# wulibingbinglin/COMET-Pose-Estimation

Hardware: AMD Instinct MI355X
Metric: sequences/sec (BxT frames) COMET fwd+bwd, T=16 512^2 (higher is better)
Workload: dtype bf16; 1 GPU; train_e2epose2.py fwd+bwd (COMET tracker+DINOv2+head, loss, backward, grad all-reduce, clip 1.0, AdamW) -- BASELINE configs[2]; global_batch=8, seq_len=16, image=512, tracks=512, parallelism=dp1

## Files before the change

### comet-pose-estimation_amd/csrc/gemm.hip

```cpp
#include <cstdio>
#include <cstdlib>
#include <type_traits>

#include "common.hpp"

namespace comet {


namespace {

constexpr int BM = 128, BN = 128, NT = 256;

struct Epi {
  const float* bias; int bias_mode; int64_t sb0, sb1;
  const void* resid; int64_t ldr, sr0, sr1; float beta;
  void* aux; int64_t ldaux, sx0, sx1;
  float alpha; int act;
  int vec;
  int wide = 0;
  int prio = 0;
  int bpark = 0;
  int raster = 0;
  const __bf16* gpre = nullptr; int64_t ldg = 0; float* dcol = nullptr;
};
// ... 527 lines not shown
    for (int e = 0; e < 4; ++e)
      if (col0 + e < N) epi_store<TC>(epi, Cb, ldc, R, X, bias, row, col0 + e, s[e]);
  }
}

template <typename TC, int NT16, int KC>
__global__ void __launch_bounds__(256)
gemm_skinny_kernel(const __bf16* __restrict__ A, int64_t lda, const __bf16* __restrict__ B, int64_t ldb,
                   TC* __restrict__ C, int64_t ldc, int64_t M, int N, int K, Epi epi) {
  const int lane = threadIdx.x & 63, li = lane & 15, g = lane >> 4;
  bf16x8 bf[NT16][KC];
#pragma unroll
  for (int nt = 0; nt < NT16; ++nt)
#pragma unroll
    for (int c = 0; c < KC; ++c) {
      const int n = nt * 16 + li, k0 = 32 * c + 8 * g;
      bf[nt][c] = (n < N && k0 < K) ? *reinterpret_cast<const bf16x8*>(B + (int64_t)n * ldb + k0) : bf16x8{};
    }
  float bias4[NT16][4];
#pragma unroll
  for (int nt = 0; nt < NT16; ++nt)
#pragma unroll
    for (int r = 0; r < 4; ++r) {
      const int n = nt * 16 + 4 * g + r;
      bias4[nt][r] = (epi.bias && n < N) ? epi.bias[n] : 0.f;
    }
  const TC* R = reinterpret_cast<const TC*>(epi.resid);
  const int64_t wave = ((int64_t)blockIdx.x * 256 + threadIdx.x) >> 6;
  const int64_t nwaves = ((int64_t)gridDim.x * 256) >> 6;
  for (int64_t m0 = wave * 16; m0 < M; m0 += nwaves * 16) {
    const int64_t m = m0 + li;
    const bool mok = m < M;
    f32x4 acc[NT16];
#pragma unroll
    for (int nt = 0; nt < NT16; ++nt) acc[nt] = f32x4{0.f, 0.f, 0.f, 0.f};
#pragma unroll
    for (int c = 0; c < KC; ++c) {
      const int k0 = 32 * c + 8 * g;
      const bf16x8 a = (mok && k0 < K) ? *reinterpret_cast<const bf16x8*>(A + m * lda + k0) : bf16x8{};
#pragma unroll
      for (int nt = 0; nt < NT16; ++nt) acc[nt] = __builtin_amdgcn_mfma_f32_16x16x32_bf16(bf[nt][c], a, acc[nt], 0, 0, 0);
    }
    if (!mok) continue;
#pragma unroll
    for (int nt = 0; nt < NT16; ++nt) {
      const int n0 = nt * 16 + 4 * g;
      if (n0 >= N) continue;
      float v[4];
#pragma unroll
      for (int r = 0; r < 4; ++r) v[r] = epi.alpha * acc[nt][r] + bias4[nt][r];
      apply_act_n<4>(epi.act, v);
      if (R) {
        float rr[4];
        load4(R + m * epi.ldr + n0, rr);
#pragma unroll
        for (int r = 0; r < 4; ++r) v[r] += epi.beta * rr[r];
      }
      store4(C + m * ldc + n0, v);
    }
  }
}

bool skinny_ok(const comet_gemm_args& a) {
  if (a.dtype_ab != COMET_BF16 || a.layout_a != 0 || a.layout_b != 0 || a.convert_a || a.convert_b) return false;
  if (a.batch[0] * a.batch[1] != 1 || a.aux != nullptr || (a.bias && a.bias_mode != 1)) return false;
  if (a.n % 16 != 0 || a.n > 64 || a.k % 8 != 0 || a.k > 256 || a.m < 16384) return false;
  const int es = a.dtype_c == COMET_F32 ? 4 : 2;
  auto al = [](const void* p, int bytes) { return p == nullptr || (uintptr_t)p % bytes == 0; };
  if (!al(a.a, 16) || a.lda % 8 != 0 || !al(a.b, 16) || a.ldb % 8 != 0) return false;
  if ((uintptr_t)a.c % (4 * es) != 0 || a.ldc % 4 != 0) return false;
  if (a.resid && ((uintptr_t)a.resid % (4 * es) != 0 || a.ldr % 4 != 0)) return false;
  return true;
}

template <typename TC>
int launch_skinny(const comet_gemm_args& a, hipStream_t s) {
  Epi e{a.bias, a.bias_mode, 0, 0, a.resid, a.ldr, 0, 0, a.beta, nullptr, 0, 0, 0, a.alpha, a.act, 0};
  const int64_t tiles = cdiv(a.m, 16);
  int64_t blocks = cdiv(tiles, 4 * 8);
  if (blocks > 4096) blocks = 4096;
  const int nt = (int)(a.n / 16), kc = (int)cdiv(a.k, 32);
#define SK(NT, KC)                                                                                          \
  hipLaunchKernelGGL((gemm_skinny_kernel<TC, NT, KC>), dim3((unsigned)blocks), dim3(256), 0, s,            \
                     (const __bf16*)a.a, a.lda, (const __bf16*)a.b, a.ldb, (TC*)a.c, a.ldc, a.m, (int)a.n, (int)a.k, e)
#define SK_K(NT) do { if (kc == 1) SK(NT, 1); else if (kc == 2) SK(NT, 2); else if (kc <= 4) SK(NT, 4); else SK(NT, 8); } while (0)
  if (nt == 1) SK_K(1); else if (nt == 2) SK_K(2); else if (nt == 3) SK_K(3); else SK_K(4);
#undef SK_K
#undef SK
  COMET_CHECK_LAUNCH("comet_gemm (skinny)");
  return COMET_OK;
}

namespace big {
constexpr int BM = 256, BK = 64, NT = 512;
constexpr int ASTAGE = BM * BK;
constexpr int CPW = 64;

typedef __attribute__((address_space(3))) void lds_void;

template <int ROWS>
__device__ __forceinline__ void glds_tile(const __bf16* __restrict__ src, int64_t ld, int64_t r0, int64_t rmax,
                                          int64_t k0, __bf16* __restrict__ img, int wid, int lane) {
  constexpr int PER_WAVE = ROWS / 8 / 8;
#pragma unroll
  for (int i = 0; i < PER_WAVE; ++i) {
    const int c = wid * PER_WAVE + i;
    const int row = c * 8 + (lane >> 3), pch = lane & 7;
    const int lch = pch ^ ((row >> 1) & 7);
    int64_t gr = r0 + row;
    gr = gr < rmax ? gr : rmax - 1;
    const __bf16* gp = src + gr * ld + k0 + lch * 8;
    __builtin_amdgcn_global_load_lds((const void*)gp, (lds_void*)(img + c * 512), 16, 0, 0);
  }
}

__device__ __forceinline__ bf16x8 frag(const __bf16* __restrict__ img, int row, int lchunk) {
  return *reinterpret_cast<const bf16x8*>(img + row * 64 + ((lchunk ^ ((row >> 1) & 7)) << 3));
}

__device__ __forceinline__ int tswz(int k) { return (k & 3) | (((k >> 3) & 1) << 2); }

template <int ROWS>
__device__ __forceinline__ void glds_tile_t(const __bf16* __restrict__ src, int64_t ld, int64_t r0, int64_t rmax,
                                            int64_t k0, __bf16* __restrict__ img, int wid, int lane) {
  constexpr int CPR = ROWS / 8;
  constexpr int KPC = 64 / CPR;
  constexpr int PER_WAVE = ROWS / 8 / 8;
#pragma unroll
  for (int i = 0; i < PER_WAVE; ++i) {
    const int c = wid * PER_WAVE + i;
    const int krow = c * KPC + lane / CPR, pch = lane % CPR;
    const int lch = pch ^ (tswz(krow) << 1);
    int64_t gr = r0 + lch * 8;
    gr = gr < rmax ? gr : rmax - 8;
    const __bf16* gp = src + (k0 + krow) * ld + gr;
    __builtin_amdgcn_global_load_lds((const void*)gp, (lds_void*)(img + c * 512), 16, 0, 0);
  }
}

typedef __attribute__((address_space(3))) s16x4 lds_s16x4g;

template <int ROWS>
__device__ __forceinline__ bf16x8 frag_t(const __bf16* __restrict__ img, int rbase, int s, int lane) {
  const int g = lane >> 4, q = (lane >> 2) & 3, p = lane & 3;
  const int u = rbase >> 4;
  const int k0 = s * 32 + 8 * g + q, k1 = k0 + 4;
  const __bf16* a0 = img + k0 * ROWS + ((u ^ tswz(k0)) << 4) + 4 * p;
  const __bf16* a1 = img + k1 * ROWS + ((u ^ tswz(k1)) << 4) + 4 * p;
  const s16x4 v0 = __builtin_amdgcn_ds_read_tr16_b64_v4i16((lds_s16x4g*)(a0));
  const s16x4 v1 = __builtin_amdgcn_ds_read_tr16_b64_v4i16((lds_s16x4g*)(a1));
  return __builtin_bit_cast(bf16x8, __builtin_shufflevector(v0, v1, 0, 1, 2, 3, 4, 5, 6, 7));
}

template <typename TC, int BN, int LA, int LB, bool SPLIT, int VAR = 0, bool DACT = false>
__global__ void __launch_bounds__(NT, 1)
gemm_big_kernel(const __bf16* __restrict__ A, int64_t lda, const __bf16* __restrict__ B, int64_t ldb,
                TC* __restrict__ C, int64_t ldc, int64_t M, int64_t N, int64_t K, int tiles_n, Epi epi,
                Split sp) {
  constexpr int WN = BN / 64, WM = 8 / WN;
  constexpr int MI = BM / WM / 16;
  constexpr int BSTAGE = BN * BK;
  constexpr int STAGING = 2 * ASTAGE + 2 * BSTAGE, PARKING = 8 * 64 * CPW * 2;
  __shared__ __attribute__((aligned(1024))) __bf16 smem[STAGING > PARKING ? STAGING : PARKING];
  const int tile = xcd_remap(blockIdx.x, gridDim.x);
  const int tm = tile / tiles_n, tn = tile % tiles_n;
  const int64_t m0 = (int64_t)tm * BM, n0 = (int64_t)tn * BN;
  const int lane = threadIdx.x & 63, wid = threadIdx.x >> 6;
  const int wr = wid / WN, wc = wid % WN;
  const int li = lane & 15, g = lane >> 4;
  __bf16* const Asm = smem;
  __bf16* const Bsm = smem + 2 * ASTAGE;

  f32x4 acc[MI][4];
#pragma unroll
  for (int i = 0; i < MI; ++i)
#pragma unroll
    for (int j = 0; j < 4; ++j) acc[i][j] = f32x4{0.f, 0.f, 0.f, 0.f};

  int64_t kbeg = 0, kend = K;
  if (SPLIT) {
    kbeg = (int64_t)blockIdx.y * sp.kchunk;
    kend = kbeg + sp.kchunk < K ? kbeg + sp.kchunk : K;
  }
  const int nk = (int)((kend - kbeg) / BK);
  auto load_tiles = [&](int64_t k0, int stage) {
    if constexpr (LA == 0) glds_tile<BM>(A, lda, m0, M, k0, Asm + stage * ASTAGE, wid, lane);
    else glds_tile_t<BM>(A, lda, m0, M, k0, Asm + stage * ASTAGE, wid, lane);
    if constexpr (LB == 0) glds_tile<BN>(B, ldb, n0, N, k0, Bsm + stage * BSTAGE, wid, lane);
    else glds_tile_t<BN>(B, ldb, n0, N, k0, Bsm + stage * BSTAGE, wid, lane);
  };
  auto afrag = [&](const __bf16* img, int rbase, int s) {
    if constexpr (LA == 0) return frag(img, rbase + li, 4 * s + g);
    else return frag_t<BM>(img, rbase, s, lane);
  };
  auto bfrag = [&](const __bf16* img, int rbase, int s) {
    if constexpr (LB == 0) return frag(img, rbase + li, 4 * s + g);
    else return frag_t<BN>(img, rbase, s, lane);
  };
  if (nk > 0) load_tiles(kbeg, 0);

  auto body = [&](int kt, auto load_next) {
    constexpr bool LOAD = decltype(load_next)::value;
    const int cur = kt & 1;
    asm volatile("s_waitcnt vmcnt(0)" ::: "memory");
    asm volatile("s_barrier" ::: "memory");
    const __bf16* a_img = Asm + cur * ASTAGE;
    const __bf16* b_img = Bsm + cur * BSTAGE;
    bf16x8 a0[MI], b0[4], a1[MI], b1[4];
    if constexpr (LOAD && VAR != 3) load_tiles(kbeg + (int64_t)(kt + 1) * BK, cur ^ 1);
#pragma unroll
    for (int j = 0; j < 4; ++j) b0[j] = bfrag(b_img, wc * 64 + j * 16, 0);
#pragma unroll
    for (int i = 0; i < MI; ++i) a0[i] = afrag(a_img, wr * (MI * 16) + i * 16, 0);
    if constexpr (LOAD && VAR == 3) load_tiles(kbeg + (int64_t)(kt + 1) * BK, cur ^ 1);
#pragma unroll
    for (int j = 0; j < 4; ++j) b1[j] = bfrag(b_img, wc * 64 + j * 16, 1);
#pragma unroll
    for (int i = 0; i < MI; ++i) a1[i] = afrag(a_img, wr * (MI * 16) + i * 16, 1);
    if constexpr (VAR == 1) __builtin_amdgcn_s_setprio(1);
#pragma unroll
    for (int i = 0; i < MI; ++i)
#pragma unroll
      for (int j = 0; j < 4; ++j)
        acc[i][j] = __builtin_amdgcn_mfma_f32_16x16x32_bf16(a0[i], b0[j], acc[i][j], 0, 0, 0);
#pragma unroll
    for (int i = 0; i < MI; ++i)
#pragma unroll
      for (int j = 0; j < 4; ++j)
        acc[i][j] = __builtin_amdgcn_mfma_f32_16x16x32_bf16(a1[i], b1[j], acc[i][j], 0, 0, 0);
    if constexpr (VAR == 1) __builtin_amdgcn_s_setprio(0);
    constexpr int RD = MI * (LA ? 2 : 1) + 4 * (LB ? 2 : 1);
    if constexpr (VAR == 3) {
      constexpr int NG = LOAD ? BM / 64 + BN / 64 : 0;
      __builtin_amdgcn_sched_group_barrier(0x100, RD, 0);
#pragma unroll
      for (int q = 0; q < NG; ++q) {
        __builtin_amdgcn_sched_group_barrier(0x020, 1, 0);
        __builtin_amdgcn_sched_group_barrier(0x008, 2, 0);
      }
#pragma unroll
      for (int q = 0; q < RD; ++q) {
        __builtin_amdgcn_sched_group_barrier(0x100, 1, 0);
        __builtin_amdgcn_sched_group_barrier(0x008, 1, 0);
      }
      __builtin_amdgcn_sched_group_barrier(0x008, 8 * MI - 2 * NG - RD, 0);
    } else if constexpr (VAR != 2) {
      constexpr int PAIRS = RD < 4 * MI ? RD : 4 * MI;
      __builtin_amdgcn_sched_group_barrier(0x100, RD, 0);
#pragma unroll
      for (int q = 0; q < PAIRS; ++q) {
        __builtin_amdgcn_sched_group_barrier(0x100, 1, 0);
        __builtin_amdgcn_sched_group_barrier(0x008, 2, 0);
      }
      __builtin_amdgcn_sched_group_barrier(0x100, RD - PAIRS, 0);
      __builtin_amdgcn_sched_group_barrier(0x008, 8 * MI - 2 * PAIRS, 0);
    }
  };
  for (int kt = 0; kt + 1 < nk; ++kt) body(kt, std::true_type{});
  if (nk > 0) body(nk - 1, std::false_type{});
  asm volatile("s_waitcnt lgkmcnt(0)" ::: "memory");
  asm volatile("s_barrier" ::: "memory");

  float* park = reinterpret_cast<float*>(smem) + wid * 64 * CPW;
  const TC* R = reinterpret_cast<const TC*>(epi.resid);
  TC* X = reinterpret_cast<TC*>(epi.aux);
  const int rq = g * 4;
  const int cg = lane & 7, rb = lane >> 3;
  const int64_t col0 = n0 + wc * 64 + cg * 8;
  float bc[8], cs[8];
#pragma unroll
  for (int e = 0; e < 8; ++e) {
    bc[e] = (epi.bias && epi.bias_mode == 1 && col0 + e < N) ? epi.bias[col0 + e] : 0.f;
    cs[e] = 0.f;
  }
#pragma unroll
  for (int h = 0; h < MI / 4; ++h) {
    if (h) asm volatile("s_waitcnt lgkmcnt(0)" ::: "memory");
#pragma unroll
    for (int i = 0; i < 4; ++i)
#pragma unroll
      for (int j = 0; j < 4; ++j)
#pragma unroll
        for (int r = 0; r < 4; ++r) {
          const int row = i * 16 + rq + r, col = j * 16 + li;
          park[row * CPW + (col ^ ((row & 3) << 4))] = acc[h * 4 + i][j][r];
        }
#pragma unroll 2
    for (int q = 0; q < 8; ++q) {
      const int rl = rb + 8 * q;
      const int64_t row = m0 + wr * (MI * 16) + h * 64 + rl;
      float v[8];
      load8(park + rl * CPW + ((cg * 8) ^ ((rl & 3) << 4)), v);
      if (row >= M || col0 >= N) continue;
      if constexpr (SPLIT) {
        float* W = sp.ws + (int64_t)blockIdx.y * M * N + row * N + col0;
        if (N % 8 == 0) {
          store8(W, v);
        } else {
#pragma unroll
          for (int e = 0; e < 8; ++e)
            if (col0 + e < N) W[e] = v[e];
        }
        continue;
      }
      if constexpr (DACT) {
        float pr[8];
        load8(epi.gpre + row * epi.ldg + col0, pr);
#pragma unroll
        for (int e = 0; e < 8; ++e) {
          const float gq = to_f32(from_f32<TC>(epi.alpha * v[e] * gelu_grad_fast(pr[e])));
          v[e] = gq;
          cs[e] += gq;
        }
        store8(C + row * ldc + col0, v);
        continue;
      }
      const float br = (epi.bias && epi.bias_mode == 2) ? epi.bias[row] : 0.f;
#pragma unroll
      for (int e = 0; e < 8; ++e) v[e] = epi.alpha * v[e] + bc[e] + br;
      if (epi.vec && col0 + 8 <= N) {
        if (X) store8(X + row * epi.ldaux + col0, v);
        apply_act_n<8>(epi.act, v);
        if (R) {
          float rr[8];
          load8(R + row * epi.ldr + col0, rr);
#pragma unroll
          for (int e = 0; e < 8; ++e) v[e] += epi.beta * rr[e];
        }
        store8(C + row * ldc + col0, v);
      } else {
#pragma unroll
        for (int e = 0; e < 8; ++e) {
          const int64_t col = col0 + e;
          if (col >= N) break;
          float o = v[e];
          if (X) X[row * epi.ldaux + col] = from_f32<TC>(o);
          o = apply_act(epi.act, o);
          if (R) o += epi.beta * to_f32(R[row * epi.ldr + col]);
          C[row * ldc + col] = from_f32<TC>(o);
        }
      }
    }
  }
  if constexpr (DACT) {
    if (epi.dcol != nullptr) {
#pragma unroll
      for (int e = 0; e < 8; ++e) {
        float x = cs[e];
        x += __shfl_xor(x, 8, 64);
        x += __shfl_xor(x, 16, 64);
        x += __shfl_xor(x, 32, 64);
        cs[e] = x;
      }
      if (rb == 0 && col0 < N) {
#pragma unroll
        for (int e = 0; e < 8; ++e) atomicAdd(epi.dcol + col0 + e, cs[e]);
      }
    }
  }
}
}

namespace w4 {
constexpr int BK = 64;
constexpr int WGM = 8;

__device__ __forceinline__ void tile_rc(int L, int tiles_m, int tiles_n, int& tm, int& tn) {
  const int gsz = WGM * tiles_n, grp = L / gsz, rem = L - grp * gsz;
  const int rows = min(WGM, tiles_m - grp * WGM);
  tm = grp * WGM + rem % rows;
  tn = rem / rows;
}

typedef __attribute__((address_space(3))) void lds_void;

constexpr int SG_MFMA = 0x008, SG_DSR = 0x100, SG_VMR = 0x020;

#ifdef COMET_GEMM_STAMPS
constexpr int ST_WG = 256, ST_TILES = 64;
__device__ unsigned long long g_stamps[ST_WG * ST_TILES * 8];
__device__ __forceinline__ void stamp(int bid, int wid, int tile, int ph) {
  const unsigned long long t = __builtin_amdgcn_s_memtime();
  if (wid == 0 && bid < ST_WG && tile < ST_TILES && (threadIdx.x & 63) == 0)
    g_stamps[((bid * ST_TILES + tile) << 3) + ph + (threadIdx.x & 63)] = t;
}
__device__ __forceinline__ void kstamp(int bid, int wid, int tile, int ph) {
  __builtin_amdgcn_sched_barrier(0);
  const unsigned long long t = __builtin_amdgcn_s_memtime();
  if ((wid == 0 || wid == 4) && bid < ST_WG && tile < 32 && (threadIdx.x & 63) == 0)
    g_stamps[((bid * ST_TILES + tile + (wid == 4 ? 32 : 0)) << 3) + ph] = t;
  __builtin_amdgcn_sched_barrier(0);
}
#define COMET_STAMP(tile, ph) stamp(bid, wid, (tile), (ph))
#define COMET_KSTAMP(tile, ph) kstamp(bid, wid, (tile), (ph))
#else
#define COMET_STAMP(tile, ph) ((void)0)
#define COMET_KSTAMP(tile, ph) ((void)0)
#endif

struct RowLN {
  __bf16* y16; int64_t ldy; float eps_y;
  __bf16* z16; int64_t ldz; const float* zw; const float* zb; float eps_z;
  int raw_c;
};

template <typename TC, int ACT, bool HASR, int NW, int TBM, int TBN, bool LN = false, bool PING = false>
__global__ void __launch_bounds__(NW * 64, 1)
gemm_w4_kernel(const __bf16* __restrict__ A, int64_t lda, const __bf16* __restrict__ B, int64_t ldb,
               TC* __restrict__ C, int64_t ldc, int64_t M, int64_t N, int64_t K, int tiles_n, int ntiles,
               Epi epi, RowLN ln) {
  constexpr int WN = NW / 2;
  constexpr int WROWS = TBM / 2;
  constexpr int WCOLS = TBN / WN;
  constexpr int MI = WROWS / 16;
  constexpr int NI = WCOLS / 16;
  constexpr int ASTAGE = TBM * BK;
  constexpr int BUF = (TBM + TBN) * BK;
  constexpr int APC = TBM / 8;
  constexpr int PA = APC >= NW ? APC / NW : 1, PB = TBN / 8 / NW;
  constexpr int NMF = MI * NI;
  constexpr int NRD = MI + NI;
  constexpr bool BPARK = std::is_same<TC, __bf16>::value && !HASR && !LN && WCOLS == 64 && ACT == COMET_ACT_NONE;
  constexpr bool PARK = std::is_same<TC, float>::value || (WCOLS % 64 == 0 && ACT == COMET_ACT_NONE && !BPARK);
  constexpr bool WIDE = !PARK && !BPARK && !HASR && std::is_same<TC, __bf16>::value && (NI % 2 == 0);
  constexpr int BSLAB = 16 * WCOLS;
  constexpr int BPARK_B = BPARK ? NW * 2 * BSLAB : 0;
  constexpr bool PSWZ = (WCOLS & (WCOLS - 1)) == 0;
  constexpr int PPITCH = PSWZ ? WCOLS : WCOLS + 4;
  constexpr int PARK_F = PARK ? NW * 8 * PPITCH : 0;
  auto pswz = [](int r) { return PSWZ ? ((r & 7) | ((r & 2) << 2)) : 0; };
  static_assert(!LN || (PARK && std::is_same<TC, float>::value), "row LN epilogue: parked f32 outputs only");
  static_assert(!LN || !BPARK, "row LN epilogue: no bf16 park");
  constexpr int STATS_F = LN ? 2 * TBM * WN : 0;
  constexpr int PARK_ELEMS = 2 * PARK_F > BPARK_B ? 2 * PARK_F : BPARK_B;
#ifdef COMET_GEMM_NO_AR
  constexpr bool AR = false;
#else
  constexpr bool AR = 2 * (3 * ASTAGE + 2 * TBN * BK + PARK_ELEMS + 2 * STATS_F) <= 160 * 1024 && TBM <= 128;
#endif
  constexpr int NA = AR ? 3 : 2;
  constexpr int BSTAGE = TBN * BK;
  constexpr int BRING = NA * ASTAGE;
  constexpr int RING = NA * ASTAGE + 2 * BSTAGE;
  constexpr int XA = AR ? PA : 0;
  static_assert(AR || RING == 2 * BUF, "ring layout");
  __shared__ __attribute__((aligned(1024))) __bf16 smem[RING + PARK_ELEMS + 2 * STATS_F];
  const int lane = threadIdx.x & 63;
  const int wid = __builtin_amdgcn_readfirstlane(threadIdx.x >> 6);
  const int wr = wid / WN, wc = wid % WN;
  const int li = lane & 15, g = lane >> 4;
  const int nk = (int)(K / BK);
  const int G = gridDim.x, bid = blockIdx.x;
  const int tiles_m = ntiles / tiles_n;
  const bool single = ntiles <= G;
  int off = single ? xcd_remap(bid, G) : (bid & 7) * (G >> 3) + (bid >> 3), strd = G, lim = ntiles;
  if (!single && epi.raster && (G & 7) == 0) {
    const int x = bid & 7, per = ntiles >> 3, rem = ntiles & 7, base = x * per + min(x, rem);
    lim = base + per + (x < rem ? 1 : 0);
    off = base + (bid >> 3);
    strd = G >> 3;
  }
  const int my_tiles = single ? 1 : (off < lim ? (lim - off + strd - 1) / strd : 0);
  const int T = my_tiles * nk;
  if (T == 0) return;

#ifdef COMET_APIECE_WRAP_ALL
  const int pieca = (wid * PA) % APC;
#else
  const int pieca = APC < NW ? (wid * PA) % APC : wid * PA;
#endif
  const int prowa = pieca * 8 + (lane >> 3), prowb = wid * PB * 8 + (lane >> 3);
  int la_it = 0, la_kt = 0, lb_it = 0, lb_kt = 0;
  const __bf16* ldA = A;
  const __bf16* ldB = B;
  int offA[PA], offB[PB];
  auto lch = [&](int r) { return ((lane & 7) ^ ((r >> 1) & 7)) * 8; };
  auto set_tile_a = [&](int it) {
    int tm, tn;
    tile_rc(off + it * strd, tiles_m, tiles_n, tm, tn);
    const int m0 = tm * TBM;
    ldA = A + (int64_t)m0 * lda;
#pragma unroll
    for (int p = 0; p < PA; ++p)
      offA[p] = (min(m0 + prowa + p * 8, (int)M - 1) - m0) * (int)lda + lch(prowa + p * 8);
  };
  auto set_tile_b = [&](int it) {
    int tm, tn;
    tile_rc(off + it * strd, tiles_m, tiles_n, tm, tn);
    const int n0 = tn * TBN;
    ldB = B + (int64_t)n0 * ldb;
#pragma unroll
    for (int p = 0; p < PB; ++p)
      offB[p] = (min(n0 + prowb + p * 8, (int)N - 1) - n0) * (int)ldb + lch(prowb + p * 8);
  };
  auto issue_a = [&](int slot) {
    const __bf16* pa = ldA + la_kt * BK;
#pragma unroll
    for (int p = 0; p < PA; ++p)
      __builtin_amdgcn_global_load_lds((const void*)(pa + offA[p]), (lds_void*)(smem + slot * ASTAGE + (pieca + p) * 512), 16, 0, 0);
  };
  auto issue_b = [&](int slot) {
    const __bf16* pb = ldB + lb_kt * BK;
#pragma unroll
    for (int p = 0; p < PB; ++p)
      __builtin_amdgcn_global_load_lds((const void*)(pb + offB[p]),
                                       (lds_void*)(smem + BRING + slot * BSTAGE + (wid * PB + p) * 512), 16, 0, 0);
  };
  auto issue_cur = [&](int aslot, int bslot) {
    if constexpr (AR) {
      issue_b(bslot);
      issue_a(aslot);
    } else {
// ... 1335 lines not shown
constexpr int PXP = CI + 8;
constexpr int MAXW = 128;
constexpr int RP = (MAXW + 2) * PXP;
typedef __attribute__((ext_vector_type(16))) float f32x16;

template <typename TC>
__global__ void __launch_bounds__(512, 1)
conv3_rows_kernel(const __bf16* __restrict__ x, int h, int w, const __bf16* __restrict__ wt, int64_t ldw,
                  TC* __restrict__ y, int64_t ldy, int64_t rows_total, int rows_per, Epi epi) {
  extern __shared__ __attribute__((aligned(16))) __bf16 lds[];
  __bf16* Ws = lds;
  __bf16* Xr = lds + CO * WP;
  constexpr int NT = 512;
  const int tid = threadIdx.x, lane = tid & 63, wid = tid >> 6;
  const int r = lane & 31, hh = lane >> 5;
  const int pb = wid & 3, cb = wid >> 2;
  const int64_t R0 = (int64_t)blockIdx.x * rows_per;
  const int64_t R1 = R0 + rows_per < rows_total ? R0 + rows_per : rows_total;
  if (R0 >= R1) return;

  for (int i = tid; i < CO * (KK / 8); i += NT) {
    const int co = i / (KK / 8), c = i % (KK / 8);
    *reinterpret_cast<uint4*>(Ws + co * WP + 8 * c) = *reinterpret_cast<const uint4*>(wt + (int64_t)co * ldw + 8 * c);
  }
  for (int i = tid; i < 4 * 2 * (CI / 8); i += NT) {
    const int slot = i / (2 * (CI / 8)), rem = i % (2 * (CI / 8));
    const int px = (rem / (CI / 8)) ? w + 1 : 0;
    *reinterpret_cast<uint4*>(Xr + slot * RP + px * PXP + 8 * (rem % (CI / 8))) = uint4{0, 0, 0, 0};
  }
  const int nch = w * (CI / 8);
  constexpr int MAXCH = MAXW * (CI / 8) / NT;
  uint4 st[MAXCH];
  auto rload = [&](int64_t ni, int row) {
    const bool in = row >= 0 && row < h;
    const __bf16* src = x + ((ni * h + (in ? row : 0)) * (int64_t)w) * CI;
#pragma unroll
    for (int i = 0; i < MAXCH; ++i) {
      const int idx = tid + i * NT;
      st[i] = (in && idx < nch) ? *reinterpret_cast<const uint4*>(src + (int64_t)idx * 8) : uint4{0, 0, 0, 0};
    }
  };
  auto rstore = [&](int row) {
    COMET_DASSERT(row >= -1 && row <= h);
    __bf16* dst = Xr + ((row + 1) & 3) * RP;
#pragma unroll
    for (int i = 0; i < MAXCH; ++i) {
      const int idx = tid + i * NT;
      if (idx < nch) *reinterpret_cast<uint4*>(dst + ((idx >> 3) + 1) * PXP + 8 * (idx & 7)) = st[i];
    }
  };
  const int px = pb * 32 + r;
  const bool pxok = px < w;
  const __bf16* wbase = Ws + (cb * 32 + r) * WP + 8 * hh;

  int64_t ni = R0 / h;
  int oy = (int)(R0 % h);
  for (int dr = -1; dr <= 1; ++dr) {
    rload(ni, oy + dr);
    rstore(oy + dr);
  }
  __syncthreads();
  for (int64_t R = R0; R < R1; ++R) {
    const bool next_same = R + 1 < R1 && oy + 1 < h;
    if (next_same) rload(ni, oy + 2);
    f32x16 acc = f32x16{};
#pragma unroll
    for (int ky = 0; ky < 3; ++ky) {
      const __bf16* xb = Xr + ((oy + ky) & 3) * RP + px * PXP + 8 * hh;
#pragma unroll
      for (int kx = 0; kx < 3; ++kx)
#pragma unroll
        for (int c = 0; c < CI; c += 16) {
          const bf16x8 bx = *reinterpret_cast<const bf16x8*>(xb + kx * PXP + c);
          const bf16x8 aw = *reinterpret_cast<const bf16x8*>(wbase + (ky * 3 + kx) * CI + c);
          acc = __builtin_amdgcn_mfma_f32_32x32x16_bf16(aw, bx, acc, 0, 0, 0);
        }
    }
    TC* yrow = y + (R * w + px) * ldy;
    const TC* rrow = reinterpret_cast<const TC*>(epi.resid) + (R * w + px) * epi.ldr;
#pragma unroll
    for (int u = 0; u < 4; u += 2) {
      float v[2][4];
#pragma unroll
      for (int e = 0; e < 2; ++e)
#pragma unroll
        for (int q = 0; q < 4; ++q) {
          const int co = 32 * cb + 8 * (u + e) + 4 * hh + q;
          v[e][q] = apply_act(epi.act, acc[4 * (u + e) + q] + (epi.bias ? epi.bias[co] : 0.f));
        }
      float o[8];
#pragma unroll
      for (int q = 0; q < 4; ++q) {
        const auto sw = __builtin_amdgcn_permlane32_swap(__float_as_uint(v[0][q]), __float_as_uint(v[1][q]), false, false);
        o[q] = __uint_as_float(sw[0]);
        o[4 + q] = __uint_as_float(sw[1]);
      }
      const int co0 = 32 * cb + 8 * u + 8 * hh;
      if (pxok) {
        if (epi.resid) {
          float rv[8];
          load8(rrow + co0, rv);
#pragma unroll
          for (int q = 0; q < 8; ++q) o[q] += epi.beta * rv[q];
        }
        store8(yrow + co0, o);
      }
    }
    if (next_same) rstore(oy + 2);
    __syncthreads();
    ++oy;
    if (oy == h && R + 1 < R1) {
      ++ni;
      oy = 0;
      for (int dr = -1; dr <= 1; ++dr) {
        rload(ni, dr);
        rstore(dr);
      }
      __syncthreads();
    }
  }
}
}

template <typename TC>
bool conv_rows_ok(const comet_conv_args& a) {
  if (getenv("COMET_CONV_NO_ROWS") != nullptr) return false;
  if (a.kh != 3 || a.kw != 3 || a.stride != 1 || a.pad != 1 || a.c != cr::CI || a.cout != cr::CO) return false;
  if (a.w > cr::MAXW || a.w < 96 || a.w % 32 != 0 || a.ldw < cr::KK || a.ldw % 8 != 0 || a.n * a.h < 256) return false;
  const uintptr_t al = 8 * sizeof(TC) >= 16 ? 16 : 8 * sizeof(TC);
  if ((uintptr_t)a.y % al != 0 || a.ldy % 8 != 0) return false;
  if (a.resid && ((uintptr_t)a.resid % al != 0 || a.ldr % 8 != 0)) return false;
  return true;
}

template <typename TC>
int launch_conv_rows(const comet_conv_args& a, hipStream_t s) {
  Epi e{a.bias, a.bias ? 1 : 0, 0, 0, a.resid, a.ldr, 0, 0, a.beta, nullptr, 0, 0, 0, 1.f, a.act, 1};
  const int64_t rows = a.n * a.h;
  int grid = num_cus();
  const int rows_per = (int)cdiv(rows, grid);
  grid = (int)cdiv(rows, rows_per);
  const size_t lds = (size_t)(cr::CO * cr::WP + 4 * cr::RP) * sizeof(__bf16);
  static bool attr = false;
  if (!attr) {
    (void)hipFuncSetAttribute((const void*)cr::conv3_rows_kernel<TC>, hipFuncAttributeMaxDynamicSharedMemorySize, (int)lds);
    attr = true;
  }
  hipLaunchKernelGGL((cr::conv3_rows_kernel<TC>), dim3((unsigned)grid), dim3(512), lds, s, (const __bf16*)a.x,
                     (int)a.h, (int)a.w, (const __bf16*)a.weight, a.ldw, (TC*)a.y, a.ldy, rows, rows_per, e);
  COMET_CHECK_LAUNCH("comet_conv2d_nhwc (3x3 rows in LDS)");
  return COMET_OK;
}

template <typename TC>
int launch_conv(const comet_conv_args& a, hipStream_t s) {
  const int64_t oh = (a.h + 2 * a.pad - a.kh) / a.stride + 1, ow = (a.w + 2 * a.pad - a.kw) / a.stride + 1;
  const int64_t M = a.n * oh * ow, N = a.cout, K = (int64_t)a.kh * a.kw * a.c;
  const int64_t tiles_m = cdiv(M, BM), tiles_n = cdiv(N, BN);
  COMET_CHECK_ARG(tiles_m * tiles_n < (1ll << 31), "comet_conv2d_nhwc: too many tiles");
  const int vec = a.cout % 8 == 0 && (uintptr_t)a.y % 32 == 0 && a.ldy % 8 == 0 &&
                  (a.resid == nullptr || ((uintptr_t)a.resid % 32 == 0 && a.ldr % 8 == 0));
  Epi e{a.bias, a.bias ? 1 : 0, 0, 0, a.resid, a.ldr, 0, 0, a.beta, nullptr, 0, 0, 0, 1.f, a.act, vec};
  bf::ConvGeo g{reinterpret_cast<const __bf16*>(a.x), (int)a.h, (int)a.w, (int)a.c, a.kw, a.stride, a.pad,
                (int)oh, (int)ow};
  if (conv_rows_ok<TC>(a)) return launch_conv_rows<TC>(a, s);
  const int64_t kcs = cdiv(K, 32);
  const bool stem = a.cout == 64 && kcs > 8 && kcs <= 13 && getenv("COMET_CONV_NO_STEM") == nullptr;
  if (a.cout % 16 == 0 && a.cout <= 64 && ((a.cout / 16) * kcs <= 32 || stem) && kcs <= 16 && M >= 16384 &&
      (uintptr_t)a.y % (4 * sizeof(TC)) == 0 && a.ldy % 4 == 0 && getenv("COMET_CONV_NO_SKINNY") == nullptr &&
      (a.resid == nullptr || ((uintptr_t)a.resid % (4 * sizeof(TC)) == 0 && a.ldr % 4 == 0)))
    return launch_conv_skinny<TC>(a, M, (int)oh, (int)ow, (int)K, s);
  Split sp{nullptr, K};
  if (N <= 64 && getenv("COMET_CONV_NO_N64") == nullptr)
    hipLaunchKernelGGL((bf::gemm_bf16_kernel<TC, 0, 0, bf::K_BF16_VEC, bf::K_BF16_VEC, false, true, true>),
                       dim3((unsigned)(tiles_m * tiles_n), 1, 1), dim3(NT), 0, s,
                       nullptr, 0, 0, 0, reinterpret_cast<const __bf16*>(a.weight), a.ldw, 0, 0,
                       reinterpret_cast<TC*>(a.y), a.ldy, 0, 0, M, N, K, 1, (int)tiles_n, e, sp, g);
  else
    hipLaunchKernelGGL((bf::gemm_bf16_kernel<TC, 0, 0, bf::K_BF16_VEC, bf::K_BF16_VEC, false, true>),
                       dim3((unsigned)(tiles_m * tiles_n), 1, 1), dim3(NT), 0, s,
                       nullptr, 0, 0, 0, reinterpret_cast<const __bf16*>(a.weight), a.ldw, 0, 0,
                       reinterpret_cast<TC*>(a.y), a.ldy, 0, 0, M, N, K, 1, (int)tiles_n, e, sp, g);
  COMET_CHECK_LAUNCH("comet_conv2d_nhwc");
  return COMET_OK;
}

}

}

extern "C" int comet_conv2d_nhwc(const comet_conv_args* args, void* stream) {
  using namespace comet;
  COMET_CHECK_ARG(args != nullptr, "comet_conv2d_nhwc: null args");
  const comet_conv_args& a = *args;
  COMET_CHECK_ARG(a.dtype == COMET_BF16, "comet_conv2d_nhwc: x/weight must be bf16 (use im2col + comet_gemm for f32)");
  COMET_CHECK_ARG(a.c > 0 && a.c % 8 == 0, "comet_conv2d_nhwc: channels must be a positive multiple of 8");
  COMET_CHECK_ARG(a.n > 0 && a.h > 0 && a.w > 0 && a.cout > 0 && a.kh > 0 && a.kw > 0 && a.stride > 0 && a.pad >= 0,
                  "comet_conv2d_nhwc: bad geometry");
  COMET_CHECK_ARG(a.h + 2 * a.pad >= a.kh && a.w + 2 * a.pad >= a.kw, "comet_conv2d_nhwc: kernel larger than padded input");
  COMET_CHECK_ARG(a.ldw >= (int64_t)a.kh * a.kw * a.c && a.ldw % 8 == 0, "comet_conv2d_nhwc: ldw < kh*kw*c or not a multiple of 8");
  COMET_CHECK_ARG(a.x && a.weight && a.y, "comet_conv2d_nhwc: null pointer");
  COMET_CHECK_ARG((uintptr_t)a.x % 16 == 0 && (uintptr_t)a.weight % 16 == 0, "comet_conv2d_nhwc: x/weight must be 16-byte aligned");
  COMET_CHECK_ARG(a.n * a.h * a.w * a.c < (1ll << 40), "comet_conv2d_nhwc: input too large");
  hipStream_t s = as_stream(stream);
  if (a.dtype_y == COMET_BF16) return launch_conv<__bf16>(a, s);
  if (a.dtype_y == COMET_F32) return launch_conv<float>(a, s);
  set_error("comet_conv2d_nhwc: bad dtype_y");
  return COMET_EINVAL;
}

extern "C" int comet_gemm_workspace(const comet_gemm_args* args, int64_t* bytes) {
  using namespace comet;
  const int rc = validate(args);
  if (rc != COMET_OK) return rc;
  COMET_CHECK_ARG(bytes != nullptr, "comet_gemm_workspace: null bytes");
  *bytes = plan_workspace(*args, make_plan(*args));
  return COMET_OK;
}

extern "C" int comet_gemm_plan(const comet_gemm_args* args, int64_t* bytes, int32_t* plan) {
  using namespace comet;
  const int rc = validate(args);
  if (rc != COMET_OK) return rc;
  COMET_CHECK_ARG(bytes != nullptr && plan != nullptr, "comet_gemm_plan: null output");
  const Plan p = make_plan(*args);
  *bytes = plan_workspace(*args, p);
  plan[0] = p.kind;
  plan[1] = p.bn;
  plan[2] = (p.kind == 3 || p.kind == 4) ? p.bm : p.splits;
  return COMET_OK;
}

static bool rowln_ok(const comet_gemm_args& a, const comet_rowln_args* ln) {
  using namespace comet;
  if (!pp_ok(a) || a.dtype_c != COMET_F32 || a.resid == nullptr || a.aux != nullptr || a.act != COMET_ACT_NONE) return false;
  if (a.n != 384 && a.n != 256) return false;
  int tbm, tbn;
  pp_tile_base(a, tbm, tbn);
  if (tbn != a.n) return false;
  auto a16 = [](const void* p) { return p == nullptr || (uintptr_t)p % 16 == 0; };
  if (!a16(a.bias)) return false;
  if (ln == nullptr) return true;
  auto b4 = [](const void* p, int64_t ld) { return p == nullptr || ((uintptr_t)p % 8 == 0 && ld % 4 == 0); };
  if (!b4(ln->y16, ln->ldy) || !b4(ln->z16, ln->ldz)) return false;
  if (ln->z16 != nullptr && (ln->zw == nullptr || ln->zb == nullptr)) return false;
  if (!a16(ln->zw) || !a16(ln->zb)) return false;
  return true;
}

extern "C" int comet_gemm_rowln_workspace(const comet_gemm_args* args, int64_t* bytes) {
  using namespace comet;
  COMET_CHECK_ARG(bytes != nullptr, "comet_gemm_rowln_workspace: null bytes");
  *bytes = 0;
  const int rc = validate(args);
  if (rc != COMET_OK) return rc;
  if (rowln_ok(*args, nullptr)) {
    if (const int sp = rowln_splits(*args)) *bytes = rowln_ws_bytes(*args, sp);
  }
  return COMET_OK;
}

extern "C" int comet_gemm_rowln_ok(const comet_gemm_args* args) {
  using namespace comet;
  if (args == nullptr || validate(args) != COMET_OK) return 0;
  return rowln_ok(*args, nullptr) ? 1 : 0;
}

extern "C" int comet_gemm_rowln(const comet_gemm_args* args, const comet_rowln_args* ln, void* stream) {
  using namespace comet;
  const int rc = validate(args);
  if (rc != COMET_OK) return rc;
  COMET_CHECK_ARG(ln != nullptr && args->a && args->b && args->c, "comet_gemm_rowln: null operand");
  COMET_CHECK_ARG(rowln_ok(*args, ln), "comet_gemm_rowln: not eligible (bf16 k-contiguous operands, K % 64 == 0, "
                                       "M >= 4096, N in {256, 384}, f32 output with a residual, no activation / aux)");
  if (args->m == 0) return COMET_OK;
  w4::RowLN r{reinterpret_cast<__bf16*>(ln->y16), ln->ldy, ln->eps_y, reinterpret_cast<__bf16*>(ln->z16), ln->ldz,
              ln->zw, ln->zb, ln->eps_z, ln->raw_c};
  return launch_pp_rowln(*args, r, as_stream(stream));
}

namespace comet {
namespace {
bool dact_ok(const comet_gemm_args& a, int act, const void* pre, int64_t ldpre) {
  if (act != COMET_ACT_GELU || a.dtype_ab != COMET_BF16 || a.dtype_c != COMET_BF16 || a.layout_a != 0) return false;
  if (a.bias || a.resid || a.aux || a.act != COMET_ACT_NONE || a.batch[0] * a.batch[1] != 1) return false;
  if (a.n % 8 != 0 || (uintptr_t)a.c % 16 != 0 || a.ldc % 8 != 0) return false;
  if (pre == nullptr || (uintptr_t)pre % 16 != 0 || ldpre % 8 != 0 || ldpre < a.n) return false;
  const Plan p = make_plan(a);
  return p.kind == 1 && p.splits == 1 && p.tail == 0 && p.bn == big_bn(a);
}

template <int BN, int LB>
int launch_big_dact(const comet_gemm_args& a, const __bf16* pre, int64_t ldpre, float* dcol, hipStream_t s) {
  Epi e{nullptr, 0, 0, 0, nullptr, 0, 0, 0, 0.f, nullptr, 0, 0, 0, a.alpha, COMET_ACT_NONE, 1};
  e.gpre = pre; e.ldg = ldpre; e.dcol = dcol;
  const int64_t tiles_m = cdiv(a.m, big::BM), tiles_n = cdiv(a.n, BN);
  COMET_CHECK_ARG(tiles_m * tiles_n < (1ll << 31), "comet_gemm_dact: too many tiles");
  if (dcol != nullptr && hipMemsetAsync(dcol, 0, a.n * sizeof(float), s) != hipSuccess) {
    set_error("comet_gemm_dact: memset failed");
    return COMET_ELAUNCH;
  }
  Split sp{nullptr, a.k};
  hipLaunchKernelGGL((big::gemm_big_kernel<__bf16, BN, 0, LB, false, 0, true>), dim3((unsigned)(tiles_m * tiles_n)),
                     dim3(big::NT), 0, s, (const __bf16*)a.a, a.lda, (const __bf16*)a.b, a.ldb, (__bf16*)a.c, a.ldc,
                     a.m, a.n, a.k, (int)tiles_n, e, sp);
  COMET_CHECK_LAUNCH("comet_gemm_dact");
  return COMET_OK;
}
}
}

extern "C" int comet_gemm_dact_ok(const comet_gemm_args* args, int32_t act, const void* pre, int64_t ldpre) {
  using namespace comet;
  if (args == nullptr || validate(args) != COMET_OK) return 0;
  return dact_ok(*args, act, pre, ldpre) ? 1 : 0;
}

extern "C" int comet_gemm_dact(const comet_gemm_args* args, int32_t act, const void* pre, int64_t ldpre, float* dbias,
                               void* stream) {
  using namespace comet;
  const int rc = validate(args);
  if (rc != COMET_OK) return rc;
  COMET_CHECK_ARG(args->a && args->b && args->c, "comet_gemm_dact: null operand");
  COMET_CHECK_ARG(dact_ok(*args, act, pre, ldpre), "comet_gemm_dact: not eligible (GELU, bf16 operands and output, "
// ... 78 lines not shown
```

Baseline: 68.87 sequences/s.

## Route large implicit-GEMM convolutions through the big-tile GEMM kernel with gather loader

Refactors the big GEMM kernel body into a reusable tile routine parameterised by a loader functor. It then adds a convolution kernel that uses the routine with an implicit-im2col gather loader (global_load_lds straight into LDS, zero line for padding), so convolutions with at least 96 output channels and large M run on the larger-tile kernel instead of the 128x128 conv GEMM. The aim is more data reuse and higher MFMA throughput for the ResNet-style convs in the tracker. In exchange the gather adds per-load index arithmetic, and the larger tiles can leave the GPU underfilled on mid-sized shapes.

```diff
diff --git a/comet-pose-estimation_amd/csrc/gemm.hip b/comet-pose-estimation_amd/csrc/gemm.hip
--- a/comet-pose-estimation_amd/csrc/gemm.hip
+++ b/comet-pose-estimation_amd/csrc/gemm.hip
@@ -703,11 +703,9 @@
   return __builtin_bit_cast(bf16x8, __builtin_shufflevector(v0, v1, 0, 1, 2, 3, 4, 5, 6, 7));
 }
 
-template <typename TC, int BN, int LA, int LB, bool SPLIT, int VAR = 0, bool DACT = false>
-__global__ void __launch_bounds__(NT, 1)
-gemm_big_kernel(const __bf16* __restrict__ A, int64_t lda, const __bf16* __restrict__ B, int64_t ldb,
-                TC* __restrict__ C, int64_t ldc, int64_t M, int64_t N, int64_t K, int tiles_n, Epi epi,
-                Split sp) {
+template <typename TC, int BN, int LA, int LB, bool SPLIT, int VAR, bool DACT, typename Load>
+__device__ __forceinline__ void big_tile(TC* __restrict__ C, int64_t ldc, int64_t M, int64_t N, int64_t kbeg, int nk,
+                                         int tiles_n, const Epi& epi, const Split& sp, Load& load) {
   constexpr int WN = BN / 64, WM = 8 / WN;
   constexpr int MI = BM / WM / 16;
   constexpr int BSTAGE = BN * BK;
@@ -728,17 +726,8 @@
 #pragma unroll
     for (int j = 0; j < 4; ++j) acc[i][j] = f32x4{0.f, 0.f, 0.f, 0.f};
 
-  int64_t kbeg = 0, kend = K;
-  if (SPLIT) {
-    kbeg = (int64_t)blockIdx.y * sp.kchunk;
-    kend = kbeg + sp.kchunk < K ? kbeg + sp.kchunk : K;
-  }
-  const int nk = (int)((kend - kbeg) / BK);
   auto load_tiles = [&](int64_t k0, int stage) {
-    if constexpr (LA == 0) glds_tile<BM>(A, lda, m0, M, k0, Asm + stage * ASTAGE, wid, lane);
-    else glds_tile_t<BM>(A, lda, m0, M, k0, Asm + stage * ASTAGE, wid, lane);
-    if constexpr (LB == 0) glds_tile<BN>(B, ldb, n0, N, k0, Bsm + stage * BSTAGE, wid, lane);
-    else glds_tile_t<BN>(B, ldb, n0, N, k0, Bsm + stage * BSTAGE, wid, lane);
+    load(k0, Asm + stage * ASTAGE, Bsm + stage * BSTAGE, m0, n0, wid, lane);
   };
   auto afrag = [&](const __bf16* img, int rbase, int s) {
     if constexpr (LA == 0) return frag(img, rbase + li, 4 * s + g);
@@ -909,6 +898,116 @@
       }
     }
   }
+}
+
+template <typename TC, int BN, int LA, int LB, bool SPLIT, int VAR = 0, bool DACT = false>
+__global__ void __launch_bounds__(NT, 1)
+gemm_big_kernel(const __bf16* __restrict__ A, int64_t lda, const __bf16* __restrict__ B, int64_t ldb,
+                TC* __restrict__ C, int64_t ldc, int64_t M, int64_t N, int64_t K, int tiles_n, Epi epi,
+                Split sp) {
+  int64_t kbeg = 0, kend = K;
+  if (SPLIT) {
+    kbeg = (int64_t)blockIdx.y * sp.kchunk;
+    kend = kbeg + sp.kchunk < K ? kbeg + sp.kchunk : K;
+  }
+  const int nk = (int)((kend - kbeg) / BK);
+  auto load = [&](int64_t k0, __bf16* a_img, __bf16* b_img, int64_t m0, int64_t n0, int wid, int lane) {
+    if constexpr (LA == 0) glds_tile<BM>(A, lda, m0, M, k0, a_img, wid, lane);
+    else glds_tile_t<BM>(A, lda, m0, M, k0, a_img, wid, lane);
+    if constexpr (LB == 0) glds_tile<BN>(B, ldb, n0, N, k0, b_img, wid, lane);
+    else glds_tile_t<BN>(B, ldb, n0, N, k0, b_img, wid, lane);
+  };
+  big_tile<TC, BN, LA, LB, SPLIT, VAR, DACT>(C, ldc, M, N, kbeg, nk, tiles_n, epi, sp, load);
+}
+
+__device__ __attribute__((aligned(128))) unsigned g_zero_line[32];
+
+template <int BN>
+struct ConvGather {
+  const __bf16* x; const __bf16* wgt; const __bf16* zero;
+  int64_t K;
+  int h, w, cin, kh, kw;
+  int64_t base[4];
+  int iy0[4], ix0[4];
+  int dy[2], dx[2], ci[2], lch[2];
+  int64_t wrow[BN / 64];
+
+  __device__ __forceinline__ ConvGather(const bf::ConvGeo& g, int kh_, const __bf16* wgt_, int64_t ldw, int64_t K_,
+                                        int64_t m0, int64_t M, int64_t n0, int64_t N, int wid, int lane)
+      : x(g.x), wgt(wgt_), zero(reinterpret_cast<const __bf16*>(g_zero_line)), K(K_), h(g.h), w(g.w), cin(g.c),
+        kh(kh_), kw(g.kw) {
+#pragma unroll
+    for (int i = 0; i < 4; ++i) {
+      const int64_t m = m0 + (wid * 4 + i) * 8 + (lane >> 3);
+      const int64_t mc = m < M ? m : M - 1;
+      const int ox = (int)(mc % g.ow);
+      const int64_t t = mc / g.ow;
+      const int oy = (int)(t % g.oh);
+      const int64_t ni = t / g.oh;
+      const int y0 = oy * g.stride - g.pad, x0 = ox * g.stride - g.pad;
+      iy0[i] = m < M ? y0 : -(1 << 30);
+      ix0[i] = x0;
+      base[i] = ((ni * g.h + y0) * g.w + x0) * g.c;
+    }
+#pragma unroll
+    for (int j = 0; j < 2; ++j) {
+      lch[j] = (lane & 7) ^ (4 * j + (lane >> 4));
+      dy[j] = 0;
+      dx[j] = 0;
+      ci[j] = 8 * lch[j];
+    }
+#pragma unroll
+    for (int i = 0; i < BN / 64; ++i) {
+      int64_t n = n0 + (wid * (BN / 64) + i) * 8 + (lane >> 3);
+      n = n < N ? n : N - 1;
+      wrow[i] = n * ldw;
+    }
+  }
+
+  __device__ __forceinline__ void operator()(int64_t k0, __bf16* a_img, __bf16* b_img, int64_t, int64_t, int wid,
+                                             int lane) {
+    int koff[2];
+    bool tap_ok[2];
+#pragma unroll
+    for (int j = 0; j < 2; ++j) {
+      koff[j] = (dy[j] * w + dx[j]) * cin + ci[j];
+      tap_ok[j] = dy[j] < kh;
+    }
+#pragma unroll
+    for (int i = 0; i < 4; ++i) {
+      const int j = i & 1;
+      const bool ok = tap_ok[j] && (unsigned)(iy0[i] + dy[j]) < (unsigned)h && (unsigned)(ix0[i] + dx[j]) < (unsigned)w;
+      const __bf16* gp = ok ? x + base[i] + koff[j] : zero;
+      __builtin_amdgcn_global_load_lds((const void*)gp, (lds_void*)(a_img + (wid * 4 + i) * 512), 16, 0, 0);
+    }
+#pragma unroll
+    for (int i = 0; i < BN / 64; ++i) {
+      const int64_t k = k0 + 8 * lch[i & 1];
+      const __bf16* gp = k < K ? wgt + wrow[i] + k : zero;
+      __builtin_amdgcn_global_load_lds((const void*)gp, (lds_void*)(b_img + (wid * (BN / 64) + i) * 512), 16, 0, 0);
+    }
+#pragma unroll
+    for (int j = 0; j < 2; ++j) {
+      ci[j] += 64;
+      const bool carry = ci[j] >= cin;
+      ci[j] -= carry ? cin : 0;
+      dx[j] += carry ? 1 : 0;
+      const bool wrap = dx[j] == kw;
+      dx[j] = wrap ? 0 : dx[j];
+      dy[j] += wrap ? 1 : 0;
+    }
+  }
+};
+
+template <typename TC, int BN>
+__global__ void __launch_bounds__(NT, 1)
+conv_big_kernel(bf::ConvGeo g, int kh, const __bf16* __restrict__ wgt, int64_t ldw, TC* __restrict__ y, int64_t ldy,
+                int64_t M, int64_t N, int64_t K, int tiles_n, Epi epi) {
+  const int tile = xcd_remap(blockIdx.x, gridDim.x);
+  const int64_t m0 = (int64_t)(tile / tiles_n) * BM, n0 = (int64_t)(tile % tiles_n) * BN;
+  ConvGather<BN> load(g, kh, wgt, ldw, K, m0, M, n0, N, threadIdx.x >> 6, threadIdx.x & 63);
+  const Split sp{nullptr, K};
+  big_tile<TC, BN, 0, 0, false, 0, false>(y, ldy, M, N, 0, (int)((K + BK - 1) / BK), tiles_n, epi, sp, load);
 }
 }
 
@@ -2550,6 +2649,29 @@
   return COMET_OK;
 }
 
+constexpr int64_t kConvBigMinM = 32768;
+int conv_big_bn(const comet_conv_args& a, int64_t M) {
+  const char* env = getenv("COMET_CONV_BIG");
+  if (env != nullptr && env[0] == '0') return 0;
+  const bool force = env != nullptr && env[0] == '1';
+  if (a.cout < 96 || a.c % 8 != 0 || a.c < 64 || a.ldw % 8 != 0) return 0;
+  if ((uintptr_t)a.x % 16 != 0 || (uintptr_t)a.weight % 16 != 0) return 0;
+  const int bn = a.cout > 128 ? 256 : 128;
+  if (!force && M < kConvBigMinM) return 0;
+  return bn;
+}
+
+template <typename TC, int BN>
+int launch_conv_big(const comet_conv_args& a, const bf::ConvGeo& g, int64_t M, int64_t K, const Epi& e, hipStream_t s) {
+  const int64_t tiles_m = cdiv(M, big::BM), tiles_n = cdiv(a.cout, BN);
+  COMET_CHECK_ARG(tiles_m * tiles_n < (1ll << 31), "comet_conv2d_nhwc: too many tiles");
+  hipLaunchKernelGGL((big::conv_big_kernel<TC, BN>), dim3((unsigned)(tiles_m * tiles_n)), dim3(big::NT), 0, s, g,
+                     (int)a.kh, reinterpret_cast<const __bf16*>(a.weight), a.ldw, reinterpret_cast<TC*>(a.y), a.ldy,
+                     M, (int64_t)a.cout, K, (int)tiles_n, e);
+  COMET_CHECK_LAUNCH("comet_conv2d_nhwc (256-row tile)");
+  return COMET_OK;
+}
+
 template <typename TC>
 int launch_conv(const comet_conv_args& a, hipStream_t s) {
   const int64_t oh = (a.h + 2 * a.pad - a.kh) / a.stride + 1, ow = (a.w + 2 * a.pad - a.kw) / a.stride + 1;
@@ -2568,6 +2690,9 @@
       (uintptr_t)a.y % (4 * sizeof(TC)) == 0 && a.ldy % 4 == 0 && getenv("COMET_CONV_NO_SKINNY") == nullptr &&
       (a.resid == nullptr || ((uintptr_t)a.resid % (4 * sizeof(TC)) == 0 && a.ldr % 4 == 0)))
     return launch_conv_skinny<TC>(a, M, (int)oh, (int)ow, (int)K, s);
+  const int big_n = conv_big_bn(a, M);
+  if (big_n == 256) return launch_conv_big<TC, 256>(a, g, M, K, e, s);
+  if (big_n == 128) return launch_conv_big<TC, 128>(a, g, M, K, e, s);
   Split sp{nullptr, K};
   if (N <= 64 && getenv("COMET_CONV_NO_N64") == nullptr)
     hipLaunchKernelGGL((bf::gemm_bf16_kernel<TC, 0, 0, bf::K_BF16_VEC, bf::K_BF16_VEC, false, true, true>),
diff --git a/profiles/conv_big/conv_big_bench.py b/profiles/conv_big/conv_big_bench.py
--- /dev/null
+++ b/profiles/conv_big/conv_big_bench.py
@@ -0,0 +1,72 @@
+import math
+import os
+import statistics
+import sys
+
+import torch
+
+ROOT = os.path.dirname(os.path.dirname(os.path.dirname(os.path.abspath(__file__))))
+sys.path.insert(0, os.path.join(ROOT, "comet-pose-estimation_amd"))
+from comet_amd import ops
+
+N = 128
+SHAPES = [("layer2.0.conv1", 1, 128, 64, 96, 3, 2, 1),
+          ("layer2.0.down", 1, 128, 64, 96, 1, 2, 0),
+          ("layer2 96->96", 3, 64, 96, 96, 3, 1, 1),
+          ("layer3.0.conv1", 1, 64, 96, 128, 3, 2, 1),
+          ("layer3.0.down", 1, 64, 96, 128, 1, 2, 0),
+          ("layer3 128->128", 3, 32, 128, 128, 3, 1, 1),
+          ("layer4.0.conv1", 1, 32, 128, 128, 3, 2, 1),
+          ("layer4.0.down", 1, 32, 128, 128, 1, 2, 0),
+          ("layer4 128->128", 3, 16, 128, 128, 3, 1, 1),
+          ("conv2", 1, 64, 416, 256, 3, 1, 1),
+          ("conv3", 1, 64, 256, 128, 1, 1, 0)]
+
+
+def timed(fn, warmup=5, calls=20):
+    for _ in range(warmup):
+        fn()
+    ts = []
+    for _ in range(calls):
+        e0, e1 = torch.cuda.Event(enable_timing=True), torch.cuda.Event(enable_timing=True)
+        e0.record()
+        fn()
+        e1.record()
+        e1.synchronize()
+        ts.append(e0.elapsed_time(e1) * 1e3)
+    return min(ts), statistics.median(ts), max(ts)
+
+
+def main():
+    total = {"old": 0.0, "new": 0.0, "default": 0.0}
+    print(f"{'shape':18s} {'M':>7s} {'K':>5s} | {'128x128 min/med/max us':>26s} TF/s | {'256-row min/med/max us':>26s} TF/s | default med us, calls per step")
+    for name, calls, hw, c, cout, k, s, p in SHAPES:
+        x = torch.randn(N, hw, hw, c, device="cuda").to(torch.bfloat16)
+        wm = (torch.randn(cout, k * k * c, device="cuda") / math.sqrt(k * k * c)).to(torch.bfloat16)
+        b = torch.randn(cout, device="cuda")
+        fn = lambda: ops.conv2d_nhwc(x, wm, k, k, s, p, bias=b, out_dtype=torch.bfloat16)
+        oh = (hw + 2 * p - k) // s + 1
+        m = N * oh * oh
+        flop = 2.0 * m * cout * k * k * c
+        res = {}
+        for tag, env in (("old", "0"), ("new", "1"), ("default", None)):
+            if env is None:
+                os.environ.pop("COMET_CONV_BIG", None)
+            else:
+                os.environ["COMET_CONV_BIG"] = env
+            res[tag] = timed(fn)
+            res[tag + "_y"] = fn().float()
+            total[tag] += calls * res[tag][1]
+        os.environ.pop("COMET_CONV_BIG", None)
+        d = (res["new_y"] - res["old_y"]).abs().max().item()
+        o, n_ = res["old"], res["new"]
+        print(f"{name:18s} {m:7d} {k * k * c:5d} | {o[0]:8.1f} {o[1]:8.1f} {o[2]:8.1f} {flop / o[1] / 1e6:5.0f} | "
+              f"{n_[0]:8.1f} {n_[1]:8.1f} {n_[2]:8.1f} {flop / n_[1] / 1e6:5.0f} | "
+              f"{res['default'][1]:8.1f}  x{calls}  max |256-row - 128x128| {d:.2e}", flush=True)
+        del x, wm
+    print(f"per step (medians x calls): 128x128 {total['old'] / 1e3:.3f} ms, 256-row {total['new'] / 1e3:.3f} ms, "
+          f"default {total['default'] / 1e3:.3f} ms")
+
+
+if __name__ == "__main__":
+    main()
```

After: 69.51 sequences/s (median of 6 runs). No clear change (+0.9%).
